# ReubenBond/DistributedRateLimiting.Redis

Hardware: AMD Instinct MI355X
Metric: acquire decisions/sec (node) at 100M keys, 1/2/4/8 GPU; % HBM roofline (higher is better)
Workload: dtype f64; 1 GPU; TokenBucket uniform keys, 2^26-request batches (config B); keys_total=100000000, keys_per_gpu=100000000, batch_per_gpu=67108864, period_ticks=10000000, partitioning=one GPU owns every key

## Files before the change

### distributedratelimiting.redis_amd/build.py

```python
from __future__ import annotations

import os
import shutil
import subprocess
import sys

HERE = os.path.dirname(os.path.realpath(__file__))
ROOT = os.path.dirname(HERE)
SOURCES = [os.path.join(HERE, "csrc", n) for n in ("tbe_engine.hip", "tbe_tools.hip", "tbe_cluster.hip", "tbe_strdir.hip")]
DEPS = SOURCES + [os.path.join(HERE, "csrc", n) for n in ("tbe_device.hpp", "tbe_codec.hpp", "tbe_numfmt.hpp", "tbe_hash.hpp", "tbe_retry.hpp", "tbe_idpool.hpp")] + \
    [os.path.join(ROOT, "include", n) for n in ("tbe.h", "tbe_tools.h", "tbe_cluster.h", "tbe_strdir.h")]
LIB = os.path.join(HERE, "libtbe.so")
ARCH = "gfx950"
HIPCC_FLAGS = ["-O3", "-std=c++17", "-ffp-contract=off", "-fno-fast-math", "-fPIC", "-shared",
               "-Wall", "-Wno-unused-result", f"--offload-arch={ARCH}"]


def hipcc() -> str:
    for cand in (os.environ.get("HIPCC"), shutil.which("hipcc"), "/opt/rocm/bin/hipcc"):
        if cand and os.path.exists(cand):
            return cand
    raise FileNotFoundError("hipcc not found")


def _digest(deps, flags) -> str:
    import hashlib
    h = hashlib.sha256(" ".join(flags).encode())
    for d in deps:
        with open(d, "rb") as f:
            h.update(os.path.basename(d).encode() + b"\0" + f.read())
    return h.hexdigest()


def up_to_date(target: str, deps, flags=()) -> bool:
    stamp = target + ".sha256"
    if not (os.path.exists(target) and os.path.exists(stamp)):
        return False
    with open(stamp) as f:
        return f.read().strip() == _digest(deps, flags)


def _stamp(target: str, deps, flags=()) -> None:
    with open(target + ".sha256", "w") as f:
# ... 44 lines not shown
```

### distributedratelimiting.redis_amd/csrc/tbe_engine.hip

```cpp
#include <hip/hip_runtime.h>

#include <algorithm>
#include <cmath>
#include <cstdarg>
#include <cstdio>
#include <cstdlib>
#include <cstring>
#include <new>
#include <string>
#include <thread>
#include <tuple>
#include <type_traits>
#include <vector>

#include "../../include/tbe.h"
#include "tbe_device.hpp"
#include "tbe_codec.hpp"
#include "tbe_numfmt.hpp"
#include "tbe_retry.hpp"

#pragma clang fp contract(off)

using namespace tbe;

namespace {

#ifndef TBE_NO_NT
#define LD_P(p) ld_nt(p)
#define ST_PERM(p, v) st_nt((p), (v))
#define LD_U(p) ld_nt(p)
#define ST_U(p, v) st_nt((p), (v))
#define ST_S(p, v) slot_store_nt((p), (v))
#else
#define LD_P(p) (*(p))
#define ST_PERM(p, v) (*(p) = (v))
#define LD_U(p) (*(p))
#define ST_U(p, v) (*(p) = (v))
#define ST_S(p, v) (*(p) = (v))
#endif
#define LD_F(p) (*(p))
#define ST_F(p, v) (*(p) = (v))

#ifndef TBE_PART_BLOCK
#define TBE_PART_BLOCK 512
#endif
#ifndef TBE_PART_ITEMS
#define TBE_PART_ITEMS 8
#endif
constexpr int kPartBlock = TBE_PART_BLOCK;
constexpr int kPartItems = TBE_PART_ITEMS;
constexpr int kTile = kPartBlock * kPartItems;
#ifndef TBE_UN_BLOCK
#define TBE_UN_BLOCK 1024
#endif
#ifndef TBE_UN_ITEMS
#define TBE_UN_ITEMS 8
#endif
constexpr int kUnBlock = TBE_UN_BLOCK;
constexpr int kUnItems = TBE_UN_ITEMS;
constexpr int kUnTile = kUnBlock * kUnItems;
#ifndef TBE_FULL_TILE
#define TBE_FULL_TILE 1
#endif
#ifndef TBE_HIST_BLOCKS
#define TBE_HIST_BLOCKS 1024
#endif
constexpr int kMaxHistBlocks = TBE_HIST_BLOCKS;
static_assert(kMaxHistBlocks % 256 == 0, "k_colscan reads kMaxHistBlocks / 256 blocks per thread");
constexpr int kMaxRBits = 11;

constexpr uint32_t kHotKeysMax = 1024;
#ifndef TBE_HOT_SLOT_BITS
#define TBE_HOT_SLOT_BITS 12
#endif
constexpr uint32_t kHotSlots = 1u << TBE_HOT_SLOT_BITS;
static_assert(kHotSlots >= 2 * kHotKeysMax, "hot table load factor <= 1/2");
constexpr uint32_t kHotEmpty = 0xFFFFFFFFu;
constexpr uint32_t kHotMin = 2048;
constexpr uint32_t kHotCandMax = 4096;

struct HotSet {
    uint32_t count;
    uint32_t n_cand;
    uint32_t key[kHotKeysMax];
    uint64_t cand[kHotCandMax];
    uint64_t slot[kHotSlots];
};

__device__ __forceinline__ uint32_t hot_hash(uint32_t key) { return (key * 0x9E3779B1u) >> (32 - TBE_HOT_SLOT_BITS); }
constexpr uint64_t kHotSlotEmpty = 0xFFFFFFFFFFFFFFFFull;
constexpr uint32_t kHotHalf = kHotSlots / 2;
__device__ __forceinline__ uint32_t hot_h1(uint32_t key) { return (key * 0x9E3779B1u) >> (33 - TBE_HOT_SLOT_BITS); }
__device__ __forceinline__ uint32_t hot_h2(uint32_t key) {
    uint32_t x = (key ^ (key >> 16)) * 0x85EBCA6Bu;
    x ^= x >> 13;
    return kHotHalf + ((x * 0xC2B2AE35u) >> (33 - TBE_HOT_SLOT_BITS));
}

constexpr uint32_t kHotLds = kHotSlots;
template <int BLOCK>
__device__ __forceinline__ bool hot_load(const HotSet *__restrict__ hot, uint64_t *slots) {
// ... 1625 lines not shown
            ST_U(retry + base + e, failed ? retry_ticks(def_in[q], rate) : (int64_t)TBE_RETRY_NONE);
        }
    }
#pragma unroll
    for (int it = 0; it < kPartItems; ++it) {
        const int e = wb_elem<kPartBlock, kPartItems>(it);
        if (e >= nvalid) continue;
        const uint64_t i = base + e;
        if (WAIT && W == 1) {
            ST_U(granted + i, (uint8_t)(r[it] >> 6));
            const uint32_t rem = r[it] & 63u;
            ST_U(remaining + i, (rem == kRemNone8) ? -1 : (int32_t)rem);
        } else if (WAIT && W == 2) {
            ST_U(granted + i, (uint8_t)(r[it] >> 14));
            const uint32_t rem = r[it] & kRemNone16;
            ST_U(remaining + i, (rem == kRemNone16) ? -1 : (int32_t)rem);
        } else if (WAIT) {
            ST_U(granted + i, (uint8_t)(r[it] >> 30));
            const uint32_t rem = r[it] & kRemNone;
            ST_U(remaining + i, (rem == kRemNone) ? -1 : (int32_t)rem);
        } else if (W == 1) {
            ST_U(granted + i, (uint8_t)(r[it] >> 7));
            ST_U(remaining + i, (int32_t)(r[it] & 0x7Fu));
        } else {
            ST_U(granted + i, (uint8_t)(r[it] >> 31));
            ST_U(remaining + i, (int32_t)(r[it] & 0x7FFFFFFFu));
        }
    }
}

#ifndef TBE_UNPART_RUNS
#define TBE_UNPART_RUNS 1
#endif
constexpr int kRunTasks1 = 3 * kPartBlock;
static_assert(kTile / 4 + 3 * kDigits / 2 <= kRunTasks1, "every run: its dwords, plus at most 1.5 for its ragged ends");
template <int W>
__global__ __launch_bounds__(kPartBlock, 8) void k_unpart_runs(
    uint64_t n, const uint16_t *__restrict__ idx, const uint32_t *__restrict__ tileprefix,
    const uint32_t *__restrict__ blockprefix, const uint32_t *__restrict__ digit_total,
    uint32_t tiles_per_blk, uint32_t ntiles, uint32_t nblk, const uint32_t *__restrict__ res_in,
    uint8_t *__restrict__ granted, int32_t *__restrict__ remaining, const uint32_t *__restrict__ err,
    uint32_t *__restrict__ sticky) {
    static_assert(W == 1 || W == 4, "one-byte or four-byte replies");
    static_assert(kTile == 8 * kPartBlock && kPartBlock >= kDigits && kPartItems == 8, "8 indices (16 bytes) per thread");
    using R = std::conditional_t<W == 1, uint8_t, uint32_t>;
    constexpr int kTasks = W == 1 ? kRunTasks1 : kTile;
    constexpr int kPer = kTasks / kPartBlock;
    __shared__ uint32_t goff[kDigits];
    __shared__ uint32_t lst[kDigits];
    __shared__ uint32_t rcnt[kDigits];
    __shared__ uint32_t tst[kDigits];
    __shared__ uint32_t wsum[kPartBlock / 64];
    __shared__ uint32_t wmax[kPartBlock / 64];
    __shared__ __attribute__((aligned(16))) uint8_t tdig[kTile];
    __shared__ __attribute__((aligned(16))) uint16_t lidx[kTile];
    __shared__ R reply[kTile];
    const int tid = threadIdx.x, lane = tid & 63, w = tid >> 6;
    if (sticky && blockIdx.x == 0 && tid == 0 && *err) *sticky = 1u;
    const uint32_t tile = xcd_swizzle(blockIdx.x, gridDim.x);
    const uint64_t base = (uint64_t)tile * kTile;
    const int nvalid = (int)min<uint64_t>(kTile, n - base);
    const u32x4 iv = LD_U(reinterpret_cast<const u32x4 *>(idx + base) + tid);
    uint32_t cnt = 0;
    if (tid < kDigits) {
        const uint32_t blk = tile / tiles_per_blk;
        const uint32_t tp = tileprefix[(uint64_t)tile * kDigits + tid];
        if (tile + 1 < ntiles && (tile + 1) % tiles_per_blk != 0) {
            cnt = tileprefix[(uint64_t)(tile + 1) * kDigits + tid] - tp;
        } else {
            const uint32_t bp = blockprefix[(uint64_t)blk * kDigits + tid];
            const uint32_t nx = blk + 1 < nblk ? blockprefix[(uint64_t)(blk + 1) * kDigits + tid] : digit_total[tid];
            cnt = nx - bp - tp;
        }
    }
    tile_offsets<kPartBlock>(tile, tiles_per_blk, tileprefix, blockprefix, digit_total, goff, wsum);
    const uint32_t g = tid < kDigits ? goff[tid] : 0u;
    const uint32_t ntask = W == 1 ? (cnt ? ((g & 3u) + cnt + 3u) >> 2 : 0u) : cnt;
    uint32_t all;
    const uint32_t sc = block_excl_scan<kPartBlock>(cnt | (ntask << 16), wsum, &all);
    const uint32_t lstart = sc & 0xFFFFu, tstart = sc >> 16;
    const uint32_t ntasks = all >> 16;
    reinterpret_cast<uint2 *>(tdig)[tid] = make_uint2(0u, 0u);
    reinterpret_cast<u32x4 *>(lidx)[tid] = iv;
    __syncthreads();
    if (tid < kDigits) {
        lst[tid] = lstart;
        rcnt[tid] = cnt;
        tst[tid] = tstart;
        if (cnt) tdig[tstart] = (uint8_t)tid;
    }
    __syncthreads();
    {
        const uint2 v = reinterpret_cast<const uint2 *>(tdig)[tid];
        uint32_t b[8];
#pragma unroll
        for (int k = 0; k < 8; ++k) b[k] = ((k < 4 ? v.x : v.y) >> (8 * (k & 3))) & 0xFFu;
#pragma unroll
        for (int k = 1; k < 8; ++k) b[k] = max(b[k], b[k - 1]);
        uint32_t inc = b[7];
#pragma unroll
        for (int o = 1; o < 64; o <<= 1) {
            const uint32_t y = __shfl_up(inc, o, 64);
            if (lane >= o) inc = max(inc, y);
        }
        uint32_t carry = __shfl_up(inc, 1, 64);
        if (lane == 0) carry = 0;
        if (lane == 63) wmax[w] = inc;
        __syncthreads();
#pragma unroll
        for (int j = 0; j < kPartBlock / 64; ++j) carry = max(carry, j < w ? wmax[j] : 0u);
        uint2 o2 = make_uint2(0u, 0u);
#pragma unroll
        for (int k = 0; k < 8; ++k) {
            const uint32_t d = max(b[k], carry);
            if (k < 4) o2.x |= d << (8 * k);
            else o2.y |= d << (8 * (k - 4));
        }
        reinterpret_cast<uint2 *>(tdig)[tid] = o2;
    }
    __syncthreads();
#pragma unroll
    for (int it = 0; it < kPer; ++it) {
        const uint32_t k = (uint32_t)(it * kPartBlock + tid);
        if (k >= ntasks) continue;
        const uint32_t d = tdig[k];
        const uint32_t gd = goff[d], t = k - tst[d];
        if constexpr (W == 1) {
            const uint32_t a = (gd & ~3u) + 4u * t;
            const uint32_t v = res_in[a >> 2];
            const uint32_t c = rcnt[d], s = lst[d];
#pragma unroll
            for (uint32_t bb = 0; bb < 4; ++bb) {
                const uint32_t p = a + bb - gd;
                if (p < c) reply[s + p] = (uint8_t)(v >> (8 * bb));
            }
        } else {
            reply[k] = res_in[gd + t];
        }
    }
    __syncthreads();
#pragma unroll
    for (int it = 0; it < kPartItems; ++it) {
        const int e = it * kPartBlock + tid;
        if (e >= nvalid) continue;
        const uint64_t i = base + e;
        const uint32_t r = reply[lidx[e] & (kTile - 1)];
        if (W == 1) {
            ST_U(granted + i, (uint8_t)(r >> 7));
            ST_U(remaining + i, (int32_t)(r & 0x7Fu));
        } else {
            ST_U(granted + i, (uint8_t)(r >> 31));
            ST_U(remaining + i, (int32_t)(r & 0x7FFFFFFFu));
        }
    }
}

constexpr int kSegBlock = kFoldBlock;
constexpr int kSegItems = 16;
constexpr uint32_t kSeg = kSegBlock * kSegItems;

struct SegSummary {
    int64_t max_ts;
    int32_t min_p;
    uint32_t pad;
};
struct SegState {
    Slot s;
    double ft;
    uint32_t pass;
    uint32_t pad;
};


__device__ __forceinline__ uint32_t seg_run(const uint32_t *segbase, uint32_t j) {
    uint32_t lo = 0, hi = kHotKeysMax;
    while (hi - lo > 1) {
        const uint32_t mid = (lo + hi) >> 1;
        if (segbase[mid] <= j) lo = mid;
        else hi = mid;
    }
    return lo;
}

template <bool SPEC>
__global__ __launch_bounds__(kSegBlock) void k_hot_summary(
    const uint64_t *__restrict__ srec, const int64_t *__restrict__ ts_orig, PackFmt F,
    const uint32_t *__restrict__ bstart, uint32_t nb, uint32_t *segbase,
// ... 1721 lines not shown
struct Workspace {
    uint64_t cap_n = 0;
    std::vector<PassBufs> pass;
    uint32_t *blocksum = nullptr;
    uint32_t *res[2] = {nullptr, nullptr};
    uint32_t *def[2] = {nullptr, nullptr};
    uint32_t *bstart = nullptr;
    uint32_t *bcount = nullptr;
    uint32_t *dlist = nullptr;
    unsigned long long *bsflags = nullptr;
    uint32_t bs_tag = 0;
    bool bs_fresh = false;
    uint8_t *dig0 = nullptr;
    uint8_t *dig1 = nullptr;
    int64_t *ts0 = nullptr;
    uint32_t *err = nullptr;
    hipEvent_t hot_done = nullptr;
    bool hot_pending = false;
    uint32_t *segbase = nullptr;
    SegSummary *summ = nullptr;
    SegState *sst = nullptr;
    hipEvent_t done = nullptr;
    bool used = false;
};

inline int ceil_log2(uint64_t x) {
    int b = 0;
    while ((1ull << b) < x) ++b;
    return b;
}

}

struct tbe_engine {
    tbe_config cfg{};
    int device = 0;
    hipStream_t stream = nullptr;
    bool own_stream = false;
    TbParams params{};
    int r_bits = 0;
    uint32_t nbuckets = 0;
    int passes = 0;
    bool packed = false;
    bool narrow = false;
    bool medium = false;
    uint32_t wait_rw() const { return narrow ? 1u : (medium ? 2u : 0u); }
    PackFmt pf{};
    bool foldrec = false;
    bool unrank = false;
    bool dig1 = false;
    bool n0 = false;
    uint32_t hot_cap = 0;
    uint32_t nb_total = 0;
    HotSet *hot[3] = {nullptr, nullptr, nullptr};
    uint64_t nbatch = 0;
    Slot *table = nullptr;
    QParams qp{};
    uint64_t *qhdr = nullptr;
    bool qh32 = false;
    uint64_t *ring = nullptr;
    uint64_t queued_total = 0;
    bool queued_exact = true;
    bool ev_pending = false;
    unsigned long long *qcount = nullptr;
    uint32_t *ev_cause = nullptr;
    int64_t *ev_id = nullptr;
    uint64_t ev_cap = 0;
    uint64_t *log_keyseq = nullptr;
    int64_t *log_id = nullptr;
// ... 91 lines not shown
        dfree(pb.digit_total);
    }
    w.pass.clear();
    dfree(w.blocksum);
    dfree(w.summ);
    dfree(w.sst);
    dfree(w.segbase);
    dfree(w.res[0]);
    dfree(w.res[1]);
    dfree(w.def[0]);
    dfree(w.def[1]);
    dfree(w.bstart);
    dfree(w.bcount);
    w.err = nullptr;
    w.dlist = nullptr;
    dfree(w.bsflags);
    dfree(w.dig0);
    dfree(w.dig1);
    dfree(w.ts0);
    w.cap_n = 0;
    w.used = false;
}

void free_staging(tbe_engine *e) {
    dfree(e->d_keys);
    dfree(e->d_permits);
    dfree(e->d_ts);
    dfree(e->d_granted);
    dfree(e->d_remaining);
    dfree(e->d_retry);
    e->stage_cap = 0;
}

void tiles_for(uint64_t n, uint32_t &ntiles, uint32_t &nblk, uint32_t &tpb) {
    ntiles = (uint32_t)((n + kTile - 1) / kTile);
    tpb = (ntiles + kMaxHistBlocks - 1) / kMaxHistBlocks;
    if (tpb == 0) tpb = 1;
    nblk = (ntiles + tpb - 1) / tpb;
}

tbe_status ensure_workspace(tbe_engine *e, Workspace &w, uint64_t n) {
    if (n <= w.cap_n) return TBE_OK;
    free_workspace(w);
    uint64_t cap = std::max<uint64_t>(n, 1u << 16);
    uint32_t ntiles, nblk, tpb;
    tiles_for(cap, ntiles, nblk, tpb);
    w.pass.resize(e->passes);
    for (auto &pb : w.pass) {
        if (e->packed) {
            HIP_TRY(e, hipMalloc(&pb.rec, cap * sizeof(uint64_t)));
        } else {
            HIP_TRY(e, hipMalloc(&pb.keys, cap * sizeof(uint32_t)));
            HIP_TRY(e, hipMalloc(&pb.permits, cap * sizeof(int32_t)));
            HIP_TRY(e, hipMalloc(&pb.ts, cap * sizeof(int64_t)));
        }
        HIP_TRY(e, hipMalloc(&pb.perm, cap * sizeof(uint32_t)));
        if (e->cfg.kind != TBE_KIND_TOKEN_BUCKET) HIP_TRY(e, hipMalloc(&pb.idx, cap * sizeof(uint32_t)));
        HIP_TRY(e, hipMalloc(&pb.tileprefix, (uint64_t)ntiles * kDigits * sizeof(uint32_t)));
        HIP_TRY(e, hipMalloc(&pb.blockprefix, (uint64_t)kMaxHistBlocks * kDigits * sizeof(uint32_t)));
        HIP_TRY(e, hipMalloc(&pb.digit_total, kDigits * sizeof(uint32_t)));
    }
    HIP_TRY(e, hipMalloc(&w.blocksum, (uint64_t)kMaxHistBlocks * kDigits * sizeof(uint32_t)));
    if (e->hot_cap) {
        const uint64_t segs = cap / kSeg + kHotKeysMax + 1;
        HIP_TRY(e, hipMalloc(&w.summ, segs * sizeof(SegSummary)));
        HIP_TRY(e, hipMalloc(&w.sst, segs * sizeof(SegState)));
        HIP_TRY(e, hipMalloc(&w.segbase, (kHotKeysMax + 1) * sizeof(uint32_t)));
    }
    HIP_TRY(e, hipMalloc(&w.res[0], cap * sizeof(uint32_t)));
    HIP_TRY(e, hipMalloc(&w.res[1], cap * sizeof(uint32_t)));
    HIP_TRY(e, hipMalloc(&w.bstart, ((uint64_t)e->nb_total + 1) * sizeof(uint32_t)));
    HIP_TRY(e, hipMalloc(&w.bcount, ((uint64_t)e->nb_total + 2 + e->nbuckets) * sizeof(uint32_t)));
    w.err = w.bcount + e->nb_total;
    w.dlist = w.bcount + e->nb_total + 1;
    HIP_TRY(e, hipMalloc(&w.bsflags, kBsMaxBlocks * sizeof(unsigned long long)));
    w.bs_fresh = true;
    w.bs_tag = 0;
    if (e->unrank) HIP_TRY(e, hipMalloc(&w.dig0, cap));
    if (e->dig1) HIP_TRY(e, hipMalloc(&w.dig1, cap));
// ... 61 lines not shown
    if (tw >= (approx ? 1 : 8)) {
        G.on = 1;
        G.n0 = (e->n0 && !(approx && e->wait_mode)) ? 1 : 0;
        G.rb = e->r_bits;
        G.pb = e->pf.pb;
        G.pw = pw;
        G.tw = tw;
        G.nb = e->nbuckets;
        G.region_bits = (uint32_t)(kDigitBits * (e->passes - 1));
        G.n_hi = (uint32_t)(((uint64_t)e->nbuckets + (1ull << G.region_bits) - 1) >> G.region_bits);
    }
    return G;
}

tbe_status run_batch(tbe_engine *e, const uint64_t *keys, const int32_t *permits,
                     const int64_t *ts, uint64_t n, uint8_t *granted, int32_t *remaining,
                     hipStream_t caller, int64_t id_base = 0, hipEvent_t in_ready = nullptr,
                     hipStream_t out_stream = nullptr, uint32_t ai_base = 0, int64_t *retry = nullptr) {
    const bool approx = e->cfg.kind == TBE_KIND_APPROXIMATE;
    const bool wait = e->cfg.kind != TBE_KIND_TOKEN_BUCKET;
    if (n == 0) return TBE_OK;
    if (n >= (1ull << 32)) return fail(e, TBE_EINVAL, "batch of %llu requests exceeds 2^32-1",
                                       (unsigned long long)n);
    if (e->packed && !approx && !ts) return fail(e, TBE_EINVAL, "null timestamps");
    const bool pipe = e->pipeline;
    Workspace &w = e->ws[pipe ? e->ws_cur : 0];
    tbe_status rc = ensure_workspace(e, w, n);
    if (rc != TBE_OK) return rc;
    if (retry) {
        if (!w.def[0]) HIP_TRY(e, hipMalloc(&w.def[0], w.cap_n * sizeof(uint32_t)));
        if (!w.def[1] && e->passes - (batch_fold_fmt(e, n).on ? 2 : 1) >= 1)
            HIP_TRY(e, hipMalloc(&w.def[1], w.cap_n * sizeof(uint32_t)));
    }
    uint32_t ntiles, nblk, tpb;
    tiles_for(n, ntiles, nblk, tpb);
    hipStream_t sf = caller ? caller : e->stream, sp = sf;
    if (pipe) {
        sf = e->stream;
        sp = e->pstream;
        if (in_ready) {
            HIP_TRY(e, hipStreamWaitEvent(sp, in_ready, 0));
        } else if (caller) {
            HIP_TRY(e, hipEventRecord(e->ev_in, caller));
            HIP_TRY(e, hipStreamWaitEvent(sp, e->ev_in, 0));
        }
        if (w.used) HIP_TRY(e, hipStreamWaitEvent(sp, w.done, 0));
        if (w.hot_pending) HIP_TRY(e, hipStreamWaitEvent(sp, w.hot_done, 0));
    } else if (in_ready) {
        HIP_TRY(e, hipStreamWaitEvent(sf, in_ready, 0));
    }
    HIP_TRY(e, hipMemsetAsync(w.bcount, 0, ((uint64_t)e->nb_total + 2) * sizeof(uint32_t), sp));
    if (w.bs_fresh) {
        HIP_TRY(e, hipMemsetAsync(w.bsflags, 0, kBsMaxBlocks * sizeof(unsigned long long), sp));
        w.bs_fresh = false;
    }

    const uint64_t kmask = e->packed ? e->pf.kmask : ~0ull;
    const FoldFmt G = batch_fold_fmt(e, n);
    PackFmt pf = e->pf;
    pf.n0 = G.n0;
    const uint64_t *rec0 = G.on ? (G.n0 ? reinterpret_cast<const uint64_t *>(w.ts0) : w.pass[e->passes - 2].rec)
                                : nullptr;
    const bool unrank = e->unrank;
    const bool runs = TBE_UNPART_RUNS && e->packed && !approx && !wait && !unrank && !retry;
    const unsigned fold_grid = G.on ? (unsigned)((1ull << G.region_bits) * G.n_hi) : e->nbuckets;
    const uint32_t tb_wmin = (!approx && !wait) ? fold_wide_min(e, n) : 1u;
    const bool sparse_tb = tb_wmin > 1u;
    const bool hot_on = e->hot_cap && !(sparse_tb && n < (1ull << TBE_HOT_SPARSE_MIN_LOG2));
    HotSet *hot = hot_on ? e->hot[e->nbatch % 3] : nullptr;
    HotSet *hot_next = hot_on ? e->hot[(e->nbatch + 2) % 3] : nullptr;
    if (hot && n >= kHotSampleMin) k_hot_sample<<<1, 1024, 0, sp>>>(keys, n, e->cfg.n_keys, hot, e->hot_cap);
    for (int p = 0; p < e->passes; ++p) {
        const int shift = e->r_bits + kDigitBits * p;
        PassBufs &out = w.pass[p];
        stage_begin(e, ST_HIST, sp);
        uint32_t *bc = (p == e->passes - 1) ? w.bcount : nullptr;
        const int lowbits = kDigitBits * p;
        uint8_t *dig = (p == 0 && unrank) ? w.dig0 : nullptr;
        uint8_t *dnext = (p == 0 && e->dig1) ? w.dig1 : nullptr;
        if (p == 0 && hot)
            k_hist<uint64_t, true><<<nblk, kHBlock, 0, sp>>>(keys, n, shift, tpb, ntiles, out.tileprefix,
                                                             w.blocksum, e->cfg.n_keys, w.err, 1, kmask,
                                                             hot, e->nbuckets, e->r_bits, bc, lowbits,
                                                             e->nb_total, dig);
        else if (p == 0)
            k_hist<uint64_t><<<nblk, kHBlock, 0, sp>>>(keys, n, shift, tpb, ntiles, out.tileprefix,
                                                       w.blocksum, e->cfg.n_keys, w.err, 1, kmask,
                                                       nullptr, e->nbuckets, e->r_bits, bc, lowbits,
                                                       e->nb_total, dig);
        else if (e->dig1 && p == 1)
            k_hist_dig<<<nblk, kHBlock, 0, sp>>>(w.dig1, n, tpb, ntiles, out.tileprefix, w.blocksum,
                                                 w.pass[0].digit_total, bc, e->nb_total);
        else if (e->packed)
            k_hist<uint64_t><<<nblk, kHBlock, 0, sp>>>(w.pass[p - 1].rec, n, shift, tpb, ntiles,
                                                       out.tileprefix, w.blocksum, e->cfg.n_keys,
                                                       w.err, 0, kmask, nullptr, e->nbuckets,
                                                       e->r_bits, bc, lowbits, e->nb_total);
        else
            k_hist<uint32_t><<<nblk, kHBlock, 0, sp>>>(w.pass[p - 1].keys, n, shift, tpb, ntiles,
                                                       out.tileprefix, w.blocksum, e->cfg.n_keys,
                                                       w.err, 0, kmask, nullptr, e->nbuckets,
                                                       e->r_bits, bc, lowbits, e->nb_total);
        stage_end(e, ST_HIST, sp);
        stage_begin(e, ST_COLSCAN, sp);
        k_colscan<<<kDigits, kBlock, 0, sp>>>(w.blocksum, nblk, out.blockprefix, out.digit_total);
        stage_end(e, ST_COLSCAN, sp);
        stage_begin(e, ST_SCATTER, sp);
// ... 219 lines not shown
            k_hot_update<<<1, 1024, 0, e->hstream>>>(hot_next, e->hot_cap - hot_reserve_host(e->hot_cap), w.err);
            HIP_TRY(e, hipEventRecord(w.hot_done, e->hstream));
            w.hot_pending = true;
        } else {
            k_hot_update<<<1, 1024, 0, sf>>>(hot_next, e->hot_cap - hot_reserve_host(e->hot_cap), w.err);
        }
        stage_end(e, ST_HOT, sf);
    }
    stage_begin(e, ST_UNSCATTER, sf);
    const unsigned untiles = (unsigned)((n + kUnTile - 1) / kUnTile);
    int cur = 0;
    for (int p = e->passes - (G.on ? 2 : 1); p >= 1; --p) {
        if (retry && e->medium)
            k_unscatter<false, false, 2, true><<<untiles, kUnBlock, 0, sf>>>(
                n, w.pass[p].perm, w.res[cur], w.res[cur ^ 1], nullptr, nullptr, nullptr, nullptr, w.def[cur],
                w.def[cur ^ 1]);
        else if (retry)
            k_unscatter<false, false, 4, true><<<untiles, kUnBlock, 0, sf>>>(
                n, w.pass[p].perm, w.res[cur], w.res[cur ^ 1], nullptr, nullptr, nullptr, nullptr, w.def[cur],
                w.def[cur ^ 1]);
        else if (e->narrow && !approx)
            k_unscatter<false, false, 1><<<untiles, kUnBlock, 0, sf>>>(n, w.pass[p].perm, w.res[cur],
                                                                   w.res[cur ^ 1], nullptr, nullptr);
        else if (e->medium)
            k_unscatter<false, false, 2><<<untiles, kUnBlock, 0, sf>>>(n, w.pass[p].perm, w.res[cur],
                                                                   w.res[cur ^ 1], nullptr, nullptr);
        else
            k_unscatter<false, false><<<untiles, kUnBlock, 0, sf>>>(n, w.pass[p].perm, w.res[cur],
                                                                    w.res[cur ^ 1], nullptr, nullptr);
        cur ^= 1;
    }
#define TBE_UNRANK(...)                                                                             \
    __VA_ARGS__<<<ntiles, kPartBlock, 0, sf>>>(n, w.dig0, w.pass[0].tileprefix, w.pass[0].blockprefix, \
                                               w.pass[0].digit_total, tpb, w.res[cur], granted, remaining)
    if (retry && unrank && e->medium)
        k_unrank<2, true, true><<<ntiles, kPartBlock, 0, sf>>>(
            n, w.dig0, w.pass[0].tileprefix, w.pass[0].blockprefix, w.pass[0].digit_total, tpb, w.res[cur],
            granted, remaining, w.def[cur], retry, e->ap.decay_rate);
    else if (retry && unrank)
        k_unrank<4, true, true><<<ntiles, kPartBlock, 0, sf>>>(
            n, w.dig0, w.pass[0].tileprefix, w.pass[0].blockprefix, w.pass[0].digit_total, tpb, w.res[cur],
            granted, remaining, w.def[cur], retry, e->ap.decay_rate);
    else if (retry && e->medium)
        k_unscatter<true, true, 2, true><<<untiles, kUnBlock, 0, sf>>>(
            n, w.pass[0].perm, w.res[cur], nullptr, granted, remaining, w.err, e->sticky, w.def[cur], nullptr,
            retry, e->ap.decay_rate);
    else if (retry)
        k_unscatter<true, true, 4, true><<<untiles, kUnBlock, 0, sf>>>(
            n, w.pass[0].perm, w.res[cur], nullptr, granted, remaining, w.err, e->sticky, w.def[cur], nullptr,
            retry, e->ap.decay_rate);
    else if (runs && e->narrow)
        k_unpart_runs<1><<<ntiles, kPartBlock, 0, sf>>>(
            n, reinterpret_cast<const uint16_t *>(w.pass[0].perm), w.pass[0].tileprefix, w.pass[0].blockprefix,
            w.pass[0].digit_total, tpb, ntiles, nblk, w.res[cur], granted, remaining, w.err, e->sticky);
    else if (runs)
        k_unpart_runs<4><<<ntiles, kPartBlock, 0, sf>>>(
            n, reinterpret_cast<const uint16_t *>(w.pass[0].perm), w.pass[0].tileprefix, w.pass[0].blockprefix,
            w.pass[0].digit_total, tpb, ntiles, nblk, w.res[cur], granted, remaining, w.err, e->sticky);
    else if (unrank && !wait && e->narrow)
        TBE_UNRANK(k_unrank<1>);
    else if (unrank && !wait)
        TBE_UNRANK(k_unrank<4>);
    else if (unrank && e->narrow)
        TBE_UNRANK(k_unrank<1, true>);
    else if (unrank && e->medium)
        TBE_UNRANK(k_unrank<2, true>);
    else if (unrank)
        TBE_UNRANK(k_unrank<4, true>);
#undef TBE_UNRANK
    else if (e->narrow && !wait && !approx)
        k_unscatter<true, false, 1><<<untiles, kUnBlock, 0, sf>>>(n, w.pass[0].perm, w.res[cur],
                                                                  nullptr, granted, remaining,
            w.err, e->sticky);
    else if (wait && e->narrow)
        k_unscatter<true, true, 1><<<untiles, kUnBlock, 0, sf>>>(n, w.pass[0].perm, w.res[cur],
                                                                 nullptr, granted, remaining,
            w.err, e->sticky);
    else if (wait && e->medium)
        k_unscatter<true, true, 2><<<untiles, kUnBlock, 0, sf>>>(n, w.pass[0].perm, w.res[cur],
                                                                 nullptr, granted, remaining,
            w.err, e->sticky);
    else if (wait)
        k_unscatter<true, true><<<untiles, kUnBlock, 0, sf>>>(n, w.pass[0].perm, w.res[cur],
                                                              nullptr, granted, remaining,
            w.err, e->sticky);
    else
        k_unscatter<true, false><<<untiles, kUnBlock, 0, sf>>>(n, w.pass[0].perm, w.res[cur],
                                                               nullptr, granted, remaining,
            w.err, e->sticky);
    stage_end(e, ST_UNSCATTER, sf);
    if (unrank) k_sticky<<<1, 64, 0, sf>>>(w.err, e->sticky);
// ... 112 lines not shown
        if (!e->packed) {
            hot_cap = 0;
            e->packed = layout(0);
        }
        e->hot_cap = hot_cap;
        e->nb_total = e->nbuckets + hot_cap;
        e->foldrec = e->packed && e->passes >= 2 && (c.flags & TBE_FLAG_UNSCATTER_ALL) == 0;
        e->unrank = e->packed && (c.flags & TBE_FLAG_UNSCATTER_ALL) == 0 && (c.flags & TBE_FLAG_RERANK) != 0;
        e->dig1 = e->packed && e->passes == 2 && (c.flags & TBE_FLAG_HIST_RECORDS) == 0;
        {
            const int w0 = 32 - e->r_bits - pbits - 1;
            e->n0 = TBE_NARROW0 && e->dig1 && e->foldrec &&
                    (c.kind == TBE_KIND_APPROXIMATE ? e->r_bits + pbits + 1 <= 32 : w0 >= 8);
            e->pf.n0 = 0;
            e->pf.rb = e->r_bits;
            e->pf.w0 = w0;
        }
        e->narrow = (c.flags & TBE_FLAG_NO_NARROW) == 0 &&
                    ((e->packed && c.kind == TBE_KIND_TOKEN_BUCKET && c.token_limit <= 127) ||
                     (c.kind == TBE_KIND_QUEUEING && c.token_limit <= 62));
        e->medium = (c.flags & TBE_FLAG_NO_NARROW) == 0 && !e->narrow && c.token_limit <= (int32_t)kRemNone16 - 1 &&
                    (c.kind == TBE_KIND_QUEUEING || c.kind == TBE_KIND_APPROXIMATE);
    }

    auto bail = [&](tbe_status st) {
        tbe_destroy(e);
        return create_fail(st, st == TBE_ENOMEM ? "device allocation failed" : "HIP device error");
    };
    if (c.device >= 0) {
        if (hipSetDevice(c.device) != hipSuccess) return bail(TBE_EDEVICE);
        e->device = c.device;
    } else if (hipGetDevice(&e->device) != hipSuccess) {
        return bail(TBE_EDEVICE);
    }
    e->pipeline = c.kind == TBE_KIND_TOKEN_BUCKET && (c.flags & TBE_FLAG_NO_PIPELINE) == 0;
    if (hipStreamCreateWithFlags(&e->stream, hipStreamNonBlocking) != hipSuccess)
        return bail(TBE_EDEVICE);
    e->own_stream = true;
    if (e->pipeline && hipStreamCreateWithFlags(&e->pstream, hipStreamNonBlocking) != hipSuccess)
        return bail(TBE_EDEVICE);
    if (e->pipeline && hipStreamCreateWithFlags(&e->hstream, hipStreamNonBlocking) != hipSuccess)
        return bail(TBE_EDEVICE);
    for (hipEvent_t *ev : {&e->ev_in, &e->ev_part, &e->ev_out, &e->ev_hot, &e->ws[0].done, &e->ws[1].done,
                           &e->ws[0].hot_done, &e->ws[1].hot_done})
        if (hipEventCreateWithFlags(ev, hipEventDisableTiming) != hipSuccess) return bail(TBE_EDEVICE);
    const uint64_t qhdr_n = (c.n_keys + 3) & ~3ull;
    uint64_t ring_n = 0;
    if (dalloc(&e->table, c.n_keys * sizeof(Slot)) != hipSuccess) return bail(TBE_ENOMEM);
    if (e->hot_cap)
        for (auto &hs : e->hot)
            if (dalloc(&hs, sizeof(HotSet)) != hipSuccess) return bail(TBE_ENOMEM);
    if (dalloc(&e->sticky, sizeof(uint32_t)) != hipSuccess) return bail(TBE_ENOMEM);
    if (c.kind == TBE_KIND_QUEUEING) {
        e->qp.token_limit = c.token_limit;
        e->qp.queue_limit = c.queue_limit;
        e->qp.order = c.queue_order;
        e->qp.cap = (uint32_t)std::max(1, c.queue_limit);
        ring_n = c.n_keys * (uint64_t)e->qp.cap;
        e->qh32 = TBE_QH32 && (uint32_t)c.queue_limit <= kQh32MaxLimit;
        if (dalloc(&e->qhdr, qhdr_n * (e->qh32 ? sizeof(uint32_t) : sizeof(uint64_t))) != hipSuccess)
            return bail(TBE_ENOMEM);
    } else if (c.kind == TBE_KIND_APPROXIMATE) {
        e->ap.token_limit = c.token_limit;
        e->ap.queue_limit = c.queue_limit;
        e->ap.order = c.queue_order;
        e->ap.zero_slots = c.zero_wait_slots;
// ... 1418 lines not shown
        cancelled[ord[c]] = hit[c];
        m += hit[c];
    }
    e->queued_total -= std::min(e->queued_total, m);
    *n_cancelled = m;
    return TBE_OK;
}

tbe_status tbe_layout(const tbe_engine *e, uint32_t *passes, uint32_t *r_bits, uint32_t *packed) {
    if (!e || !passes || !r_bits || !packed) return TBE_EINVAL;
    *passes = (uint32_t)e->passes;
    *r_bits = (uint32_t)e->r_bits;
    *packed = (e->packed ? 1u : 0u) | (e->hot_cap ? 2u : 0u) | (e->pipeline ? 4u : 0u) |
              (e->narrow ? 8u : 0u) | (e->medium ? 16u : 0u) | (e->foldrec ? 32u : 0u) |
              (e->dig1 ? 64u : 0u) | (e->unrank ? 128u : 0u) | (e->n0 ? 256u : 0u) | (e->qh32 ? 512u : 0u);
    return TBE_OK;
}

tbe_status tbe_batch_format(const tbe_engine *e, uint64_t n, uint32_t *out, uint32_t n_out) {
    if (!e || !out || n_out < 8) return TBE_EINVAL;
    const FoldFmt G = batch_fold_fmt(e, n);
    out[0] = (uint32_t)e->passes;
    out[1] = (uint32_t)G.on;
    out[2] = (uint32_t)G.pw;
    out[3] = (uint32_t)G.tw;
    out[4] = (uint32_t)e->pf.kb;
    out[5] = (uint32_t)e->pf.pb;
    out[6] = (uint32_t)(G.n0 ? e->pf.w0 : e->pf.wb);
    out[7] = (uint32_t)e->r_bits;
    if (n_out > 8) {
        const bool tb = e->cfg.kind == TBE_KIND_TOKEN_BUCKET;
        out[8] = (tb && fold_wide_min(e, n) > 1u) ? 1u : 0u;
    }
    return TBE_OK;
}

tbe_status tbe_stage_times(tbe_engine *e, double *out, uint32_t n_out, uint32_t *n_written) {
    if (!e || !out || !n_written) return TBE_EINVAL;
    double ms_sum[ST_COUNT] = {};
    if (!e->ev_marks.empty()) {
        HIP_TRY(e, hipSetDevice(e->device));
        HIP_TRY(e, hipEventSynchronize(e->ev_pool[e->ev_marks.back().second + 1]));
        for (const auto &m : e->ev_marks) {
            float ms = 0.f;
            HIP_TRY(e, hipEventElapsedTime(&ms, e->ev_pool[m.second], e->ev_pool[m.second + 1]));
            ms_sum[m.first] += ms;
        }
    }
    e->ev_marks.clear();
    e->ev_used = 0;
    const uint32_t m = std::min<uint32_t>(n_out, ST_COUNT);
    for (uint32_t i = 0; i < m; ++i) out[i] = ms_sum[i];
    *n_written = m;
    return TBE_OK;
}

}
```

### distributedratelimiting.redis_amd/engine.py

```python
from __future__ import annotations

import ctypes
from ctypes import byref, c_double, c_int32, c_uint32, c_void_p
from typing import Optional, Tuple

import numpy as np

from . import _capi
from ._capi import TbeError


def fill_rate(tokens_per_period: int, period_ticks: int) -> float:
    return _capi.load().tbe_fill_rate(tokens_per_period, period_ticks)


class PinnedArray:

    def __init__(self, n: int, dtype):
        self._lib = _capi.load()
        dt = np.dtype(dtype)
        nbytes = max(1, int(n) * dt.itemsize)
        p = c_void_p()
        st = self._lib.tbe_alloc_host(nbytes, byref(p))
        if st != 0 or not p.value:
# ... 155 lines not shown
        self._check(self._lib.tbe_export_live_device(self.handle, ts_us, first, count, None, None, None, 0,
                                                     d_n.data_ptr(), stream))
        torch.cuda.synchronize(dev)
        n = int(d_n.item())
        d_ids = torch.empty(n, dtype=torch.int64, device=dev)
        d_v = torch.empty(n, dtype=torch.float64, device=dev)
        d_t = torch.empty(n, dtype=torch.int64, device=dev)
        if n:
            self._check(self._lib.tbe_export_live_device(self.handle, ts_us, first, count, d_ids.data_ptr(),
                                                         d_v.data_ptr(), d_t.data_ptr(), n, d_n.data_ptr(), stream))
            if not stream:
                torch.cuda.synchronize(dev)
        return d_ids, d_v, d_t

    def import_rows(self, d_ids, d_v, d_t_us, stream: Optional[int] = None) -> None:
        n = d_ids.numel()
        if d_v.numel() != n or d_t_us.numel() != n:
            raise ValueError("d_ids, d_v and d_t_us must have the same length")
        d_ids, d_v, d_t_us = d_ids.contiguous(), d_v.contiguous(), d_t_us.contiguous()
        self._check(self._lib.tbe_import_rows_device(self.handle, d_ids.data_ptr(), d_v.data_ptr(),
                                                     d_t_us.data_ptr(), n, stream))
        self._rows_in_flight = (d_ids, d_v, d_t_us)

    def layout(self) -> dict:
        a, b, c = c_uint32(), c_uint32(), c_uint32()
        self._check(self._lib.tbe_layout(self.handle, byref(a), byref(b), byref(c)))
        return {"passes": a.value, "r_bits": b.value, "packed": bool(c.value & 1),
                "hot": bool(c.value & 2), "pipeline": bool(c.value & 4), "narrow": bool(c.value & 8),
                "medium": bool(c.value & 16), "fold_records": bool(c.value & 32),
                "digit_stream": bool(c.value & 64), "rerank": bool(c.value & 128),
                "narrow_pass0": bool(c.value & 256), "queue_header_32": bool(c.value & 512)}

    def batch_format(self, n: int) -> dict:
        out = (c_uint32 * 9)()
        self._check(self._lib.tbe_batch_format(self.handle, n, out, 9))
        names = ("passes", "fold_records", "position_bits", "fold_time_bits", "key_bits", "permit_bits",
                 "pass0_time_bits", "r_bits", "sparse")
        return {k: (bool(out[i]) if k in ("fold_records", "sparse") else out[i]) for i, k in enumerate(names)}

    def stage_times(self) -> dict:
        out = (c_double * len(_capi.STAGES))()
        nw = c_uint32()
        self._check(self._lib.tbe_stage_times(self.handle, out, len(_capi.STAGES), byref(nw)))
        return {name: out[i] for i, name in enumerate(_capi.STAGES[: nw.value])}


class QueueingTokenBucketEngine(TokenBucketEngine):

    KIND = _capi.TBE_KIND_QUEUEING

    def __init__(self, n_keys: int, token_limit: int, tokens_per_period: int, period_ticks: int,
                 queue_limit: int, queue_order: int = 0, **kw):
        super().__init__(n_keys, token_limit, tokens_per_period, period_ticks,
                         queue_limit=queue_limit, queue_order=queue_order, **kw)
        self.queue_limit = queue_limit

    def wait_batch(self, keys, permits, ts_us, id_base: int, status=None, remaining=None):
        keys = np.ascontiguousarray(keys, dtype=np.uint64)
        permits = np.ascontiguousarray(permits, dtype=np.int32)
        ts_us = np.ascontiguousarray(ts_us, dtype=np.int64)
        n = keys.shape[0]
        status = np.empty(n, dtype=np.uint8) if status is None else status
        remaining = np.empty(n, dtype=np.int32) if remaining is None else remaining
        n_ev = ctypes.c_uint64()
        self._check(self._lib.tbe_wait_batch(self.handle, keys.ctypes.data, permits.ctypes.data,
                                             ts_us.ctypes.data, n, id_base, status.ctypes.data,
                                             remaining.ctypes.data, byref(n_ev)))
        m = n_ev.value
        cause = np.empty(m, dtype=np.uint64)
        ids = np.empty(m, dtype=np.int64)
        nw = ctypes.c_uint64()
# ... 255 lines not shown
```

Baseline: 44.55 billion decisions/s.

## Vectorize unpart_runs reply stores and add occupancy-sized histogram grids

The k_unpart_runs epilogue now has each thread gather its own 8 replies by tile index. When the outputs are aligned and the tile is full, it writes them as one 64-bit granted store and two 128-bit remaining stores instead of strided scalar stores, and the lidx shared array is dropped. Separately, a per-pass histogram grid sizing is added: it can round the block count to a multiple of the 8 XCDs, and when TBE_HIST_ROUND is set it caps blocks to occupancy×CU count. It also reports the grids through batch_format. The hist rounding is off by default, but the multiple-of-8 rounding of the 1024 cap is a no-op, so the main active change is the wider, coalesced per-thread output writes.

```diff
diff --git a/distributedratelimiting.redis_amd/build.py b/distributedratelimiting.redis_amd/build.py
--- a/distributedratelimiting.redis_amd/build.py
+++ b/distributedratelimiting.redis_amd/build.py
@@ -8,7 +8,7 @@
 HERE = os.path.dirname(os.path.realpath(__file__))
 ROOT = os.path.dirname(HERE)
 SOURCES = [os.path.join(HERE, "csrc", n) for n in ("tbe_engine.hip", "tbe_tools.hip", "tbe_cluster.hip", "tbe_strdir.hip")]
-DEPS = SOURCES + [os.path.join(HERE, "csrc", n) for n in ("tbe_device.hpp", "tbe_codec.hpp", "tbe_numfmt.hpp", "tbe_hash.hpp", "tbe_retry.hpp", "tbe_idpool.hpp")] + \
+DEPS = SOURCES + [os.path.join(HERE, "csrc", n) for n in ("tbe_device.hpp", "tbe_codec.hpp", "tbe_numfmt.hpp", "tbe_hash.hpp", "tbe_retry.hpp", "tbe_idpool.hpp", "tbe_tiles.hpp")] + \
     [os.path.join(ROOT, "include", n) for n in ("tbe.h", "tbe_tools.h", "tbe_cluster.h", "tbe_strdir.h")]
 LIB = os.path.join(HERE, "libtbe.so")
 ARCH = "gfx950"
diff --git a/distributedratelimiting.redis_amd/csrc/tbe_engine.hip b/distributedratelimiting.redis_amd/csrc/tbe_engine.hip
--- a/distributedratelimiting.redis_amd/csrc/tbe_engine.hip
+++ b/distributedratelimiting.redis_amd/csrc/tbe_engine.hip
@@ -18,6 +18,7 @@
 #include "tbe_codec.hpp"
 #include "tbe_numfmt.hpp"
 #include "tbe_retry.hpp"
+#include "tbe_tiles.hpp"
 
 #pragma clang fp contract(off)
 
@@ -67,6 +68,9 @@
 #endif
 constexpr int kMaxHistBlocks = TBE_HIST_BLOCKS;
 static_assert(kMaxHistBlocks % 256 == 0, "k_colscan reads kMaxHistBlocks / 256 blocks per thread");
+#ifndef TBE_HIST_ROUND
+#define TBE_HIST_ROUND 0
+#endif
 constexpr int kMaxRBits = 11;
 
 constexpr uint32_t kHotKeysMax = 1024;
@@ -1758,6 +1762,9 @@
 #ifndef TBE_UNPART_RUNS
 #define TBE_UNPART_RUNS 1
 #endif
+#ifndef TBE_UNPART_WIDE
+#define TBE_UNPART_WIDE 1
+#endif
 constexpr int kRunTasks1 = 3 * kPartBlock;
 static_assert(kTile / 4 + 3 * kDigits / 2 <= kRunTasks1, "every run: its dwords, plus at most 1.5 for its ragged ends");
 template <int W>
@@ -1779,7 +1786,9 @@
     __shared__ uint32_t wsum[kPartBlock / 64];
     __shared__ uint32_t wmax[kPartBlock / 64];
     __shared__ __attribute__((aligned(16))) uint8_t tdig[kTile];
+#if !TBE_UNPART_WIDE
     __shared__ __attribute__((aligned(16))) uint16_t lidx[kTile];
+#endif
     __shared__ R reply[kTile];
     const int tid = threadIdx.x, lane = tid & 63, w = tid >> 6;
     if (sticky && blockIdx.x == 0 && tid == 0 && *err) *sticky = 1u;
@@ -1807,7 +1816,9 @@
     const uint32_t lstart = sc & 0xFFFFu, tstart = sc >> 16;
     const uint32_t ntasks = all >> 16;
     reinterpret_cast<uint2 *>(tdig)[tid] = make_uint2(0u, 0u);
+#if !TBE_UNPART_WIDE
     reinterpret_cast<u32x4 *>(lidx)[tid] = iv;
+#endif
     __syncthreads();
     if (tid < kDigits) {
         lst[tid] = lstart;
@@ -1865,6 +1876,39 @@
         }
     }
     __syncthreads();
+#if TBE_UNPART_WIDE
+    {
+        const int e0 = 8 * tid;
+        uint32_t r[8];
+#pragma unroll
+        for (int k = 0; k < 8; ++k) r[k] = reply[(iv[k >> 1] >> (16 * (k & 1))) & (kTile - 1)];
+        constexpr int kGShift = W == 1 ? 7 : 31;
+        constexpr uint32_t kRMask = W == 1 ? 0x7Fu : 0x7FFFFFFFu;
+        const bool al = ((reinterpret_cast<uintptr_t>(granted) & 7u) | (reinterpret_cast<uintptr_t>(remaining) & 15u)) == 0;
+        if (al && e0 + 8 <= nvalid) {
+            uint64_t g8 = 0;
+            u32x4 lo, hi;
+#pragma unroll
+            for (int k = 0; k < 8; ++k) {
+                g8 |= (uint64_t)(r[k] >> kGShift) << (8 * k);
+                if (k < 4) lo[k] = r[k] & kRMask;
+                else hi[k - 4] = r[k] & kRMask;
+            }
+            ST_U(reinterpret_cast<uint64_t *>(granted + base + e0), g8);
+            ST_U(reinterpret_cast<u32x4 *>(remaining + base + e0), lo);
+            ST_U(reinterpret_cast<u32x4 *>(remaining + base + e0) + 1, hi);
+        } else {
+#pragma unroll
+            for (int k = 0; k < 8; ++k) {
+                if (e0 + k < nvalid) {
+                    const uint64_t i = base + e0 + k;
+                    ST_U(granted + i, (uint8_t)(r[k] >> kGShift));
+                    ST_U(remaining + i, (int32_t)(r[k] & kRMask));
+                }
+            }
+        }
+    }
+#else
 #pragma unroll
     for (int it = 0; it < kPartItems; ++it) {
         const int e = it * kPartBlock + tid;
@@ -1879,6 +1923,7 @@
             ST_U(remaining + i, (int32_t)(r & 0x7FFFFFFFu));
         }
     }
+#endif
 }
 
 constexpr int kSegBlock = kFoldBlock;
@@ -3666,9 +3711,12 @@
 
 }
 
+enum HistKind { HK_HOT = 0, HK_U64, HK_U32, HK_DIG, HK_COUNT };
+
 struct tbe_engine {
     tbe_config cfg{};
     int device = 0;
+    uint32_t hist_slots[HK_COUNT] = {kMaxHistBlocks, kMaxHistBlocks, kMaxHistBlocks, kMaxHistBlocks};
     hipStream_t stream = nullptr;
     bool own_stream = false;
     TbParams params{};
@@ -3826,19 +3874,22 @@
     e->stage_cap = 0;
 }
 
-void tiles_for(uint64_t n, uint32_t &ntiles, uint32_t &nblk, uint32_t &tpb) {
-    ntiles = (uint32_t)((n + kTile - 1) / kTile);
-    tpb = (ntiles + kMaxHistBlocks - 1) / kMaxHistBlocks;
-    if (tpb == 0) tpb = 1;
-    nblk = (ntiles + tpb - 1) / tpb;
+int hist_kind(const tbe_engine *e, int p, bool hot) {
+    if (p == 0) return hot ? HK_HOT : HK_U64;
+    if (e->dig1 && p == 1) return HK_DIG;
+    return e->packed ? HK_U64 : HK_U32;
+}
+
+void pass_grid(const tbe_engine *e, uint64_t n, int p, bool hot, uint32_t &ntiles, uint32_t &nblk, uint32_t &tpb) {
+    const uint32_t slots = TBE_HIST_ROUND ? e->hist_slots[hist_kind(e, p, hot)] : (uint32_t)kMaxHistBlocks;
+    tiles_for(n, kTile, slots, kMaxHistBlocks, ntiles, nblk, tpb);
 }
 
 tbe_status ensure_workspace(tbe_engine *e, Workspace &w, uint64_t n) {
     if (n <= w.cap_n) return TBE_OK;
     free_workspace(w);
     uint64_t cap = std::max<uint64_t>(n, 1u << 16);
-    uint32_t ntiles, nblk, tpb;
-    tiles_for(cap, ntiles, nblk, tpb);
+    const uint32_t ntiles = (uint32_t)((cap + kTile - 1) / kTile);
     w.pass.resize(e->passes);
     for (auto &pb : w.pass) {
         if (e->packed) {
@@ -3966,8 +4017,7 @@
         if (!w.def[1] && e->passes - (batch_fold_fmt(e, n).on ? 2 : 1) >= 1)
             HIP_TRY(e, hipMalloc(&w.def[1], w.cap_n * sizeof(uint32_t)));
     }
-    uint32_t ntiles, nblk, tpb;
-    tiles_for(n, ntiles, nblk, tpb);
+    const uint32_t ntiles = (uint32_t)((n + kTile - 1) / kTile);
     hipStream_t sf = caller ? caller : e->stream, sp = sf;
     if (pipe) {
         sf = e->stream;
@@ -4004,9 +4054,13 @@
     HotSet *hot = hot_on ? e->hot[e->nbatch % 3] : nullptr;
     HotSet *hot_next = hot_on ? e->hot[(e->nbatch + 2) % 3] : nullptr;
     if (hot && n >= kHotSampleMin) k_hot_sample<<<1, 1024, 0, sp>>>(keys, n, e->cfg.n_keys, hot, e->hot_cap);
+    uint32_t nt0, nblk0, tpb0;
+    pass_grid(e, n, 0, hot != nullptr, nt0, nblk0, tpb0);
     for (int p = 0; p < e->passes; ++p) {
         const int shift = e->r_bits + kDigitBits * p;
         PassBufs &out = w.pass[p];
+        uint32_t ntp, nblk, tpb;
+        pass_grid(e, n, p, hot != nullptr, ntp, nblk, tpb);
         stage_begin(e, ST_HIST, sp);
         uint32_t *bc = (p == e->passes - 1) ? w.bcount : nullptr;
         const int lowbits = kDigitBits * p;
@@ -4292,14 +4346,14 @@
     }
 #define TBE_UNRANK(...)                                                                             \
     __VA_ARGS__<<<ntiles, kPartBlock, 0, sf>>>(n, w.dig0, w.pass[0].tileprefix, w.pass[0].blockprefix, \
-                                               w.pass[0].digit_total, tpb, w.res[cur], granted, remaining)
+                                               w.pass[0].digit_total, tpb0, w.res[cur], granted, remaining)
     if (retry && unrank && e->medium)
         k_unrank<2, true, true><<<ntiles, kPartBlock, 0, sf>>>(
-            n, w.dig0, w.pass[0].tileprefix, w.pass[0].blockprefix, w.pass[0].digit_total, tpb, w.res[cur],
+            n, w.dig0, w.pass[0].tileprefix, w.pass[0].blockprefix, w.pass[0].digit_total, tpb0, w.res[cur],
             granted, remaining, w.def[cur], retry, e->ap.decay_rate);
     else if (retry && unrank)
         k_unrank<4, true, true><<<ntiles, kPartBlock, 0, sf>>>(
-            n, w.dig0, w.pass[0].tileprefix, w.pass[0].blockprefix, w.pass[0].digit_total, tpb, w.res[cur],
+            n, w.dig0, w.pass[0].tileprefix, w.pass[0].blockprefix, w.pass[0].digit_total, tpb0, w.res[cur],
             granted, remaining, w.def[cur], retry, e->ap.decay_rate);
     else if (retry && e->medium)
         k_unscatter<true, true, 2, true><<<untiles, kUnBlock, 0, sf>>>(
@@ -4312,11 +4366,11 @@
     else if (runs && e->narrow)
         k_unpart_runs<1><<<ntiles, kPartBlock, 0, sf>>>(
             n, reinterpret_cast<const uint16_t *>(w.pass[0].perm), w.pass[0].tileprefix, w.pass[0].blockprefix,
-            w.pass[0].digit_total, tpb, ntiles, nblk, w.res[cur], granted, remaining, w.err, e->sticky);
+            w.pass[0].digit_total, tpb0, ntiles, nblk0, w.res[cur], granted, remaining, w.err, e->sticky);
     else if (runs)
         k_unpart_runs<4><<<ntiles, kPartBlock, 0, sf>>>(
             n, reinterpret_cast<const uint16_t *>(w.pass[0].perm), w.pass[0].tileprefix, w.pass[0].blockprefix,
-            w.pass[0].digit_total, tpb, ntiles, nblk, w.res[cur], granted, remaining, w.err, e->sticky);
+            w.pass[0].digit_total, tpb0, ntiles, nblk0, w.res[cur], granted, remaining, w.err, e->sticky);
     else if (unrank && !wait && e->narrow)
         TBE_UNRANK(k_unrank<1>);
     else if (unrank && !wait)
@@ -4495,6 +4549,21 @@
         e->device = c.device;
     } else if (hipGetDevice(&e->device) != hipSuccess) {
         return bail(TBE_EDEVICE);
+    }
+    if (TBE_HIST_ROUND) {
+        int cus = 0;
+        if (hipDeviceGetAttribute(&cus, hipDeviceAttributeMultiprocessorCount, e->device) != hipSuccess)
+            return bail(TBE_EDEVICE);
+        auto slots_of = [&](auto kernel, uint32_t &slots) {
+            int per_cu = 0;
+            if (hipOccupancyMaxActiveBlocksPerMultiprocessor(&per_cu, kernel, kHBlock, 0) != hipSuccess) return false;
+            const int64_t s = (int64_t)per_cu * cus;
+            slots = (uint32_t)std::min<int64_t>(std::max<int64_t>(s, 1), kMaxHistBlocks);
+            return true;
+        };
+        if (!slots_of(k_hist<uint64_t, true>, e->hist_slots[HK_HOT]) || !slots_of(k_hist<uint64_t>, e->hist_slots[HK_U64]) ||
+            !slots_of(k_hist<uint32_t>, e->hist_slots[HK_U32]) || !slots_of(k_hist_dig, e->hist_slots[HK_DIG]))
+            return bail(TBE_EDEVICE);
     }
     e->pipeline = c.kind == TBE_KIND_TOKEN_BUCKET && (c.flags & TBE_FLAG_NO_PIPELINE) == 0;
     if (hipStreamCreateWithFlags(&e->stream, hipStreamNonBlocking) != hipSuccess)
@@ -5979,6 +6048,12 @@
         const bool tb = e->cfg.kind == TBE_KIND_TOKEN_BUCKET;
         out[8] = (tb && fold_wide_min(e, n) > 1u) ? 1u : 0u;
     }
+    const bool sparse_tb = e->cfg.kind == TBE_KIND_TOKEN_BUCKET && fold_wide_min(e, n) > 1u;
+    const bool hot = e->hot_cap && !(sparse_tb && n < (1ull << TBE_HOT_SPARSE_MIN_LOG2));
+    for (int p = 0; p < e->passes && 9u + 2u * p + 1u < n_out; ++p) {
+        uint32_t ntiles;
+        pass_grid(e, n, p, hot, ntiles, out[9 + 2 * p], out[10 + 2 * p]);
+    }
     return TBE_OK;
 }
 
diff --git a/distributedratelimiting.redis_amd/csrc/tbe_tiles.hpp b/distributedratelimiting.redis_amd/csrc/tbe_tiles.hpp
--- /dev/null
+++ b/distributedratelimiting.redis_amd/csrc/tbe_tiles.hpp
@@ -0,0 +1,20 @@
+#pragma once
+
+#include <cstdint>
+
+namespace tbe {
+
+constexpr uint32_t kXcds = 8;
+
+inline void tiles_for(uint64_t n, uint32_t tile, uint32_t slots, uint32_t max_blocks, uint32_t &ntiles,
+                      uint32_t &nblk, uint32_t &tpb) {
+    ntiles = (uint32_t)((n + tile - 1) / tile);
+    uint32_t cap = slots < max_blocks ? slots : max_blocks;
+    if (cap >= kXcds) cap -= cap % kXcds;
+    if (cap == 0) cap = 1;
+    tpb = (ntiles + cap - 1) / cap;
+    if (tpb == 0) tpb = 1;
+    nblk = (ntiles + tpb - 1) / tpb;
+}
+
+}
diff --git a/distributedratelimiting.redis_amd/engine.py b/distributedratelimiting.redis_amd/engine.py
--- a/distributedratelimiting.redis_amd/engine.py
+++ b/distributedratelimiting.redis_amd/engine.py
@@ -211,11 +211,13 @@
                 "narrow_pass0": bool(c.value & 256), "queue_header_32": bool(c.value & 512)}
 
     def batch_format(self, n: int) -> dict:
-        out = (c_uint32 * 9)()
-        self._check(self._lib.tbe_batch_format(self.handle, n, out, 9))
+        out = (c_uint32 * 17)()
+        self._check(self._lib.tbe_batch_format(self.handle, n, out, 17))
         names = ("passes", "fold_records", "position_bits", "fold_time_bits", "key_bits", "permit_bits",
                  "pass0_time_bits", "r_bits", "sparse")
-        return {k: (bool(out[i]) if k in ("fold_records", "sparse") else out[i]) for i, k in enumerate(names)}
+        d = {k: (bool(out[i]) if k in ("fold_records", "sparse") else out[i]) for i, k in enumerate(names)}
+        d["hist_grid"] = [(out[9 + 2 * p], out[10 + 2 * p]) for p in range(min(out[0], 4))]
+        return d
 
     def stage_times(self) -> dict:
         out = (c_double * len(_capi.STAGES))()
```

New measurement: 44.79 billion decisions/s (median of 6 runs). About the same (+0.5%).
